# azmyrajab/polars_ols

Hardware: AMD Instinct MI355X
Metric: group_regressions_per_sec (higher is better)
Workload: dtype f32

## Files before the change

polars_ols_amd/csrc/api.hip:

```cpp
#include <algorithm>
#include <cmath>
#include <cctype>
#include <cstdlib>
#include <strings.h>
#include <condition_variable>
#include <mutex>
#include <thread>

#include "common.hpp"
#include "api_internal.hpp"
#include "k1_gram_chol.hpp"
#include "k2_resident.hpp"
#include "k2w_resident.hpp"
#include "k4_rolling.hpp"
#include "k5_enet.hpp"
#include "k6_svd.hpp"
#include "k8_wide.hpp"
#include "k10_ridge_path.hpp"
#include "k11_rlm.hpp"
#include "k13_glm.hpp"
#include "k14_iv.hpp"
#include "k12_enet_cv.hpp"
#include "dyn_prep.hpp"

// ... 118 lines not shown
    const uint64_t sum = ((h0 * 31 + h1) * 31 + h2) * 31 + h3;
    const bool hit = ctx->offsets.valid && ctx->offs_n == n_groups && ctx->offs_sum == sum &&
                     ctx->offs_copy.size() == (size_t)cnt && std::memcmp(ctx->offs_copy.data(), offs, bytes) == 0;
    if (!hit) {
        void *dptr = nullptr;
        ctx->offsets.valid = false;
        int rc = grow(ctx->offsets, bytes, &dptr);
        if (rc) return rc;
        if ((rc = upload_small(ctx, dptr, offs, bytes))) return rc;
        ctx->offsets.valid = true;
        ctx->offs_copy.assign(offs, offs + cnt);
        ctx->offs_n = n_groups;
        ctx->offs_sum = sum;
        ctx->offs_id++;
    }
    ctx->offs_host = offs;
    ctx->offs_generation = generation;
    ctx->offs_max_rows = sc.max_rows;
    ctx->offs_min_rows = sc.min_rows;
    ctx->offs_small_mask = sc.small_mask;
    std::memcpy(ctx->offs_hist_cnt, sc.hist_cnt, sizeof(sc.hist_cnt));
    std::memcpy(ctx->offs_hist_rows, sc.hist_rows, sizeof(sc.hist_rows));
    ctx->offs_wave_overflow = sc.wave_overflow;
    ctx->offs_tail_group = sc.tail_group;
    ctx->offs_aligned[0] = sc.aligned[0];
    ctx->offs_aligned[1] = sc.aligned[1];
    *d_offs = static_cast<const int64_t *>(ctx->offsets.buf.ptr);
    *max_rows = sc.max_rows;
    return POLS_OK;
}

static bool ieq(const char *a, const char *b) {
    for (; *a && *b; ++a, ++b)
        if (std::tolower((unsigned char)*a) != std::tolower((unsigned char)*b)) return false;
    return *a == *b;
}

bool options_set(Options &o, const char *key, const char *v) {
    if (!key) return false;
    if (!strncasecmp(key, "POLS_", 5)) key += 5;
    const bool on = v != nullptr;
    const Options d;
    if (ieq(key, "TIMELINE")) o.timeline = on;
    else if (ieq(key, "K1_NOOCC4")) o.k1_noocc4 = on;
    else if (ieq(key, "K1_NOFAST")) o.k1_nofast = on;
    else if (ieq(key, "K1_NOEDGE")) o.k1_noedge = on;
    else if (ieq(key, "K1_NOTINY")) o.k1_notiny = on;
    else if (ieq(key, "K1_NORC1")) o.k1_norc1 = on;
    else if (ieq(key, "K1_SHAPE")) { o.k1_shape_team = on && ieq(v, "team"); o.k1_shape_wave = on && ieq(v, "wave"); }
    else if (ieq(key, "K1_F64_TEAM")) o.k1_f64_team256 = on && std::atoi(v) == 256;
    else if (ieq(key, "KG_NOYV")) o.kg_noyv = on;
    else if (ieq(key, "KG_SINGLE_BUFFER")) o.kg_single_buffer = on;
    else if (ieq(key, "NO_CLASSES")) o.no_classes = on;
    else if (ieq(key, "PREDICT_LOOP")) o.predict_loop = on;
    else if (ieq(key, "K2_NOPREFETCH")) o.k2_noprefetch = on;
    else if (ieq(key, "NO_SPLIT")) o.no_split = on;
    else if (ieq(key, "K1_PASSES")) o.k1_passes = on ? std::atoi(v) : d.k1_passes;
    else if (ieq(key, "K1_WG")) o.k1_wg = on ? std::atoi(v) : d.k1_wg;
    else if (ieq(key, "K1T_RC4")) o.k1t_rc4 = on ? (std::atoi(v) != 0) : d.k1t_rc4;
    else if (ieq(key, "K1T_SUB8")) o.k1t_sub8 = on ? std::atoi(v) : d.k1t_sub8;
    else if (ieq(key, "K1_NT_LOADS")) o.k1_nt_loads = on ? (std::atoi(v) != 0) : d.k1_nt_loads;
    else if (ieq(key, "K1_XCD")) o.k1_xcd = on ? std::atoi(v) : d.k1_xcd;
    else if (ieq(key, "K4P_LPS")) o.k4p_lps = on ? std::atoi(v) : d.k4p_lps;
    else if (ieq(key, "SEG_TARGET")) o.seg_target = on ? std::atoi(v) : d.seg_target;
    else if (ieq(key, "K1_RC2_WIDE")) o.k1_rc2_wide = on ? std::atoi(v) != 0 : d.k1_rc2_wide;
    else if (ieq(key, "DEBUG_SKIP_FIXUP")) o.debug_skip_fixup = on && std::atoi(v) != 0;
    else if (ieq(key, "K1_PERSIST")) o.k1_persist = on ? (std::atoi(v) != 0) : d.k1_persist;
    else if (ieq(key, "K1_PERSIST_SUB")) o.k1_persist_sub = on ? std::atoi(v) : d.k1_persist_sub;
    else if (ieq(key, "K1T_SUB32")) o.k1t_sub32 = on ? (std::atoi(v) != 0) : d.k1t_sub32;
    else if (ieq(key, "STATIC_ENGINE")) o.static_engine = !on ? 0 : ieq(v, "stream") ? 1 : ieq(v, "k2") ? 2 : ieq(v, "nok2") ? 3 : ieq(v, "k2w") ? 4 : 0;
    else if (ieq(key, "RLS_ENGINE")) o.rls_engine = !on ? RlsEngine::Auto : ieq(v, "seq") ? RlsEngine::Seq : ieq(v, "scan") ? RlsEngine::Scan : ieq(v, "chunk") ? RlsEngine::Chunk : ieq(v, "halo") ? RlsEngine::Halo : RlsEngine::Auto;
    else if (ieq(key, "RLM_ENGINE")) o.rlm_engine = !on ? 0 : ieq(v, "stream") ? 1 : 0;
    else if (ieq(key, "GLM_ENGINE")) o.glm_engine = !on ? 0 : ieq(v, "split") ? 1 : 0;
    else if (ieq(key, "ABSORB2_ROUTE")) o.absorb2_route = !on ? 0 : ieq(v, "global") ? 1 : 0;
    else if (ieq(key, "RANDOM_EFFECTS_ROUTE")) o.random_effects_route = !on ? 0 : ieq(v, "global") ? 1 : 0;
    else if (ieq(key, "RLS_SPINS")) o.rls_spin_limit = on ? std::atoi(v) : d.rls_spin_limit;
    else if (ieq(key, "RLS_EARLY")) o.rls_early = on ? std::atoi(v) : d.rls_early;
    else if (ieq(key, "ROLLING_ENGINE")) {
        using E = RollingEngine;
        o.rolling_engine = !on ? E::Auto : ieq(v, "chunk") ? E::Chunk : ieq(v, "halo") ? E::Halo : ieq(v, "nocompact") ? E::NoCompact : ieq(v, "halowave") ? E::HaloWave : ieq(v, "scatter") ? E::Scatter : E::Auto;
    }
    else if (ieq(key, "K1_ENGINE")) o.k1_engine = !on ? 0 : ieq(v, "valu") ? 1 : ieq(v, "mfma") ? 2 : 0;
    else if (ieq(key, "K9_TAKE")) o.k9_take = !on ? 0 : ieq(v, "gather") ? 1 : ieq(v, "scatter") ? 2 : 0;
    else return false;
    return true;
}

void options_from_env(Options &o) {
    static const char *const keys[] = {"TIMELINE", "K1_NOOCC4", "K1_NOFAST", "K1_NOTINY", "K1_NORC1", "K1_SHAPE", "K1_F64_TEAM",
                                       "KG_NOYV", "K2_NOPREFETCH", "K1_PASSES", "K1_WG", "RLS_SPINS", "RLS_EARLY", "K1T_RC4", "K1_NT_LOADS", "STATIC_ENGINE",
                                       "RLS_ENGINE", "RLM_ENGINE", "GLM_ENGINE", "ABSORB2_ROUTE", "RANDOM_EFFECTS_ROUTE", "ROLLING_ENGINE", "K1_ENGINE", "K9_TAKE", "K1_PERSIST", "K1_PERSIST_SUB", "K1T_SUB32", "K1_NOEDGE", "K1T_SUB8",
                                       "K1_XCD", "NO_SPLIT", "DEBUG_SKIP_FIXUP", "K4P_LPS", "SEG_TARGET", "K1_RC2_WIDE", "KG_SINGLE_BUFFER", "PREDICT_LOOP", "NO_CLASSES"};
    char name[64];
    for (const char *k : keys) {
        std::snprintf(name, sizeof(name), "POLS_%s", k);
        if (const char *v = std::getenv(name)) options_set(o, k, v);
    }
}

static bool timing_sampled(pols_ctx *ctx) {
    if (!ctx->timing) return false;
    return (ctx->timing_tick++ % ctx->timing_stride) == 0;
}

void timing_begin(pols_ctx *ctx) {
    ctx->timing_open = false;
    if (!timing_sampled(ctx)) return;
    ctx->timing_open = true;
    if (ctx->timed_used == ctx->timed.size()) {
        TimedLaunch t;
        if (hipEventCreate(&t.start) != hipSuccess || hipEventCreate(&t.stop) != hipSuccess) return;
        ctx->timed.push_back(t);
    }
    hipEventRecord(ctx->timed[ctx->timed_used].start, ctx->stream);
}

bool timing_pair(pols_ctx *ctx, hipEvent_t *start, hipEvent_t *stop) {
    if (!timing_sampled(ctx)) return false;
    if (ctx->timed_used == ctx->timed.size()) {
        TimedLaunch t;
        if (hipEventCreate(&t.start) != hipSuccess || hipEventCreate(&t.stop) != hipSuccess) return false;
        ctx->timed.push_back(t);
    }
    *start = ctx->timed[ctx->timed_used].start;
    *stop = ctx->timed[ctx->timed_used].stop;
    ctx->timed_used++;
    return true;
}

void timing_end(pols_ctx *ctx) {
    if (!ctx->timing_open || ctx->timed_used >= ctx->timed.size()) return;
    ctx->timing_open = false;
    hipEventRecord(ctx->timed[ctx->timed_used].stop, ctx->stream);
    ctx->timed_used++;
}

int check_ctx(pols_ctx *ctx) {
    if (!ctx) return fail(POLS_ERR_INVALID, "ctx is NULL");
    POLS_HIP(hipSetDevice(ctx->device));
    return POLS_OK;
}


template <typename T>
__global__ void __launch_bounds__(256) null_weights_kernel(const T *w, T *out, int64_t n) {
    using V = typename Vec16<T>::type;
    constexpr int VN = Vec16<T>::N;
    const int64_t i0 = ((int64_t)blockIdx.x * 256 + threadIdx.x) * VN;
    if (i0 + VN <= n) {
        const V v = *reinterpret_cast<const V *>(w + i0);
        T f[4];
#pragma unroll
        for (int e = 0; e < VN; ++e) { const T x = vget<T>(v, e); f[e] = x != x ? (T)1e-24 : x; }
        if constexpr (VN == 4) *reinterpret_cast<V *>(out + i0) = V{f[0], f[1], f[2], f[3]};
        else *reinterpret_cast<V *>(out + i0) = V{f[0], f[1]};
    } else {
        for (int64_t i = i0; i < n; ++i) { const T x = w[i]; out[i] = x != x ? (T)1e-24 : x; }
    }
}

int fill_null_weights(pols_ctx *ctx, const pols_batch *b, Staged *st) {
    if (!st->w || b->null_free || b->n_rows <= 0) return POLS_OK;
    void *dst = const_cast<void *>(st->w);
    if (b->mem == POLS_MEM_DEVICE) {
        int rc = ensure_scratch(ctx, Work::NullWeights, round256(dtype_size(b->dtype) * (size_t)b->n_rows), &dst);
        if (rc) return rc;
    }
    const int vn = b->dtype == POLS_F32 ? 4 : 2;
    const unsigned blocks = (unsigned)((b->n_rows + 256 * (int64_t)vn - 1) / (256 * (int64_t)vn));
    if (b->dtype == POLS_F32) hipLaunchKernelGGL(null_weights_kernel<float>, dim3(blocks), dim3(256), 0, ctx->stream, static_cast<const float *>(st->w), static_cast<float *>(dst), b->n_rows);
    else hipLaunchKernelGGL(null_weights_kernel<double>, dim3(blocks), dim3(256), 0, ctx->stream, static_cast<const double *>(st->w), static_cast<double *>(dst), b->n_rows);
    POLS_HIP(hipGetLastError());
    st->w = dst;
    return POLS_OK;
// ... 170 lines not shown
    if (same_frame) extra_per_seg = std::max<size_t>(extra_per_seg, sc.nz2);
    sc.valid = false;
    std::vector<int64_t> so;
    std::vector<int32_t> sm, sf((size_t)n_items + 1);
    if (!ids) so.push_back(0);
    int64_t max_len = 0, max_seg = 0;
    for (int64_t i = 0; i < n_items; ++i) {
        const int64_t g = ids ? (int64_t)(*ids)[(size_t)i] : i;
        if (i > 0) max_seg = std::max<int64_t>(max_seg, (int64_t)sm.size() - sf[(size_t)i - 1]);
        sf[(size_t)i] = (int32_t)sm.size();
        const int64_t s0 = b->group_offsets[g], e0 = b->group_offsets[g + 1];
        const int64_t pieces = std::max<int64_t>(1, (e0 - s0 + seg_target - 1) / seg_target);
        const int64_t len = std::max<int64_t>(1, ((e0 - s0 + pieces - 1) / pieces + 255) / 256 * 256);
        max_len = std::max(max_len, std::min(len, e0 - s0));
        for (int64_t r = s0; r < e0 || r == s0; r += len) {
            if (ids) so.push_back(r);
            so.push_back(std::min(e0, r + len));
            sm.push_back((int32_t)i);
            if (e0 == s0) break;
        }
    }
    sf[(size_t)n_items] = (int32_t)sm.size();
    if (n_items > 0) max_seg = std::max<int64_t>(max_seg, (int64_t)sm.size() - sf[(size_t)n_items - 1]);
    const int64_t n_seg = (int64_t)sm.size();
    seg_tables_layout(cv, *t, n_seg, n_items, ids != nullptr, extra_per_seg);
    if ((rc = carve(sc, cv))) return rc;
    if ((rc = upload_small(ctx, const_cast<int64_t *>(t->offs), so.data(), sizeof(int64_t) * so.size()))) return rc;
    if ((rc = upload_small(ctx, const_cast<int32_t *>(t->map), sm.data(), sizeof(int32_t) * sm.size()))) return rc;
    if ((rc = upload_small(ctx, const_cast<int32_t *>(t->first), sf.data(), sizeof(int32_t) * sf.size()))) return rc;
    sc.valid = true; sc.offs_id = ctx->offs_id; sc.n_groups = b->n_groups; sc.n_rows = b->n_rows; sc.seg_target = seg_target;
    sc.class_key = class_key; sc.n_items = n_items;
    sc.n_seg = n_seg; sc.nz2 = extra_per_seg; sc.nulls = false; sc.max_len = max_len; sc.max_seg = max_seg;
    t->max_len = max_len; t->max_seg = max_seg;
    return POLS_OK;
}

extern "C" {

int pols_device_count(void) {
    int n = 0;
    if (hipGetDeviceCount(&n) != hipSuccess) return 0;
    return n;
}

const char *pols_version(void) { return "pols_mi355x 0.1.0 (gfx950)"; }
const char *pols_last_error(void) { return g_err; }

int pols_create(int device_id, pols_ctx **out) {
    if (!out) return fail(POLS_ERR_INVALID, "out is NULL");
    *out = nullptr;
    int n = 0;
    if (hipGetDeviceCount(&n) != hipSuccess || n <= 0)
        return fail(POLS_ERR_NO_DEVICE, "no HIP device visible; libpols_mi355x has no CPU fallback");
    if (device_id < 0 || device_id >= n) return fail(POLS_ERR_INVALID, "device_id %d out of range [0, %d)", device_id, n);
    POLS_HIP(hipSetDevice(device_id));
    hipDeviceProp_t prop;
    POLS_HIP(hipGetDeviceProperties(&prop, device_id));
    if (std::strncmp(prop.gcnArchName, "gfx950", 6) != 0)
        return fail(POLS_ERR_NO_DEVICE, "device %d is %s; this library carries gfx950 code objects only", device_id, prop.gcnArchName);
    pols_ctx *ctx = new pols_ctx();
    ctx->device = device_id;
    ctx->num_cus = prop.multiProcessorCount;
    if (hipStreamCreateWithFlags(&ctx->own_stream, hipStreamNonBlocking) != hipSuccess) {
        delete ctx;
        return fail(POLS_ERR_HIP, "hipStreamCreate failed");
    }
    ctx->stream = ctx->own_stream;
    options_from_env(ctx->opt);
    *out = ctx;
    return POLS_OK;
}

int pols_set_option(pols_ctx *ctx, const char *key, const char *value) {
    if (!ctx || !key) return fail(POLS_ERR_INVALID, "ctx / key is NULL");
    if (!options_set(ctx->opt, key, value)) return fail(POLS_ERR_INVALID, "unknown option '%s'", key);
    return POLS_OK;
}

void pols_destroy(pols_ctx *ctx) {
    if (!ctx) return;
    hipSetDevice(ctx->device);
    hipStreamSynchronize(ctx->stream);
    for (DeviceBuffer *d : {&ctx->offsets.buf, &ctx->chunk_cache.buf, &ctx->k3c.buf, &ctx->k3h.buf, &ctx->class_cache.buf, &ctx->seg_cache[0].buf,
                            &ctx->seg_cache[1].buf, &ctx->start_flags.buf, &ctx->k3c_gran, &ctx->k4c_fix})
        if (d->ptr) hipFree(d->ptr);
    for (auto &d : ctx->work)
        if (d.ptr) hipFree(d.ptr);
    if (ctx->fb_flag) hipFree(ctx->fb_flag);
    for (auto &t : ctx->timed) { hipEventDestroy(t.start); hipEventDestroy(t.stop); }
    for (auto &ps : ctx->pinned) {
        if (ps.done) hipEventDestroy(ps.done);
        if (ps.ptr) hipHostFree(ps.ptr);
    }
    if (ctx->switch_event) hipEventDestroy(ctx->switch_event);
    if (ctx->own_stream) hipStreamDestroy(ctx->own_stream);
    delete ctx;
}

int pols_set_stream(pols_ctx *ctx, void *hip_stream) {
    if (!ctx) return fail(POLS_ERR_INVALID, "ctx is NULL");
    hipStream_t next = static_cast<hipStream_t>(hip_stream);
    if (next != ctx->stream) {
        if (!ctx->switch_event) POLS_HIP(hipEventCreateWithFlags(&ctx->switch_event, hipEventDisableTiming));
        POLS_HIP(hipEventRecord(ctx->switch_event, ctx->stream));
        POLS_HIP(hipStreamWaitEvent(next, ctx->switch_event, 0));
    }
    ctx->stream = next;
    return POLS_OK;
}

int pols_use_private_stream(pols_ctx *ctx) {
    if (!ctx) return fail(POLS_ERR_INVALID, "ctx is NULL");
    return pols_set_stream(ctx, ctx->own_stream);
}

int pols_synchronize(pols_ctx *ctx) {
    int rc = check_ctx(ctx);
    if (rc) return rc;
    POLS_HIP(hipStreamSynchronize(ctx->stream));
    return POLS_OK;
}

int pols_timing_enable(pols_ctx *ctx, int enable) {
    if (!ctx) return fail(POLS_ERR_INVALID, "ctx is NULL");
    ctx->timing = enable != 0;
    ctx->timing_stride = enable > 1 ? enable : 1;
    ctx->timing_tick = 0;
    ctx->timed_used = 0;
    return POLS_OK;
}

int pols_timing_collect(pols_ctx *ctx, float *ms_out, int max) {
    if (!ctx || !ms_out) return fail(POLS_ERR_INVALID, "NULL argument");
    if (hipStreamSynchronize(ctx->stream) != hipSuccess) return fail(POLS_ERR_HIP, "stream sync failed");
    int n = 0;
    for (size_t i = 0; i < ctx->timed_used && n < max; ++i) {
        float ms = 0.f;
        if (hipEventElapsedTime(&ms, ctx->timed[i].start, ctx->timed[i].stop) == hipSuccess) ms_out[n++] = ms;
    }
    ctx->timed_used = 0;
    return n;
}

const char *pols_last_kernel_name(pols_ctx *ctx) { return ctx ? ctx->last_kernel.c_str() : ""; }

void pols_ols_params_default(pols_ols_params *p) {
    std::memset(p, 0, sizeof(*p));
    p->alpha = 0.0;
    p->has_l1_ratio = 0;
    p->max_iter = 1000;
    p->tol = 1.0e-5;
    p->positive = 0;
    p->solve_method = POLS_SOLVE_AUTO;
    p->has_rcond = 0;
    p->null_policy = POLS_NULL_IGNORE;
}

int pols_predict(pols_ctx *ctx, const pols_batch *b, const void *coef, int64_t coef_rows, void *pred_out) {
    return pols_predict_policy(ctx, b, coef, coef_rows, POLS_NULL_IGNORE, pred_out);
}

int pols_predict_policy(pols_ctx *ctx, const pols_batch *b, const void *coef, int64_t coef_rows, int32_t null_policy, void *pred_out) {
    int rc = check_ctx(ctx);
    if (rc) return rc;
    pols_out o;
    std::memset(&o, 0, sizeof(o));
    o.pred = pred_out;
// ... 276 lines not shown
```

polars_ols_amd/csrc/api_static.hip:

```cpp
#include <algorithm>
#include <cmath>
#include <cstring>
#include <string>

#include "common.hpp"
#include "api_internal.hpp"
#include "k1_gram_chol.hpp"
#include "k2_resident.hpp"
#include "k2w_resident.hpp"
#include "k5_enet.hpp"
#include "k6_svd.hpp"
#include "k8_wide.hpp"
#include "../../include/pols_mi355x_debug.h"

namespace pols {
template <typename T> bool k1m_fits(int k_user, bool has_w, int64_t max_rows);

int resolve_solve_plan(const pols_ols_params *p, int dtype, int kt, int n_targets, SolvePlan *out) {
    const int m = p->solve_method;
    const double alpha = p->alpha;
    const bool positive = p->positive != 0, multi = n_targets > 1;
    SolvePlan s;
    if (alpha == 0.0 && !positive && (m == POLS_SOLVE_AUTO || m == POLS_SOLVE_SVD || m == POLS_SOLVE_QR)) {
        s.branch = SolveBranch::Ols;
// ... 476 lines not shown
    if (!p) return fail(POLS_ERR_INVALID, "params is NULL");
    StaticCall c{ctx, b, p, o};
    if ((rc = effective_null_policy(b, p, &c.pol))) return rc;
    c.kt = b->n_features + (b->add_intercept ? 1 : 0);
    if ((rc = resolve_solve_plan(p, b->dtype, c.kt, 1, &c.plan))) return rc;
    if (b->n_groups == 0) return POLS_OK;
    if (c.kt > 31) {
        if (info) return fail(POLS_ERR_INVALID, "internal: the wide statistics path calls wide_static itself");
        return wide_static(ctx, b, p, o, c.kt, c.plan);
    }
    if ((rc = upload_offsets(ctx, b->group_offsets, b->n_groups, &c.d_offs, &c.max_rows, b->offsets_generation))) return rc;
    if ((rc = stage_inputs(ctx, b, b->n_groups, c.kt, o, &c.st))) return rc;
    if ((rc = fill_null_weights(ctx, b, &c.st))) return rc;
    if (!c.plan.enet()) {
        if (!c.st.status) {
            void *sp = nullptr;
            if ((rc = ensure_scratch(ctx, Work::Status, sizeof(int32_t) * (size_t)b->n_groups, &sp))) return rc;
            c.st.status = static_cast<int32_t *>(sp);
        }
        if ((rc = ensure_fallback_epoch(ctx))) return rc;
    }
    const RoutePick r = pick_static_route(route_inputs(ctx->opt, b, p, c.pol, c.plan, c.max_rows, ctx->offs_aligned, ctx->offs_hist_cnt, ctx->offs_hist_rows));
    switch (r.route) {
        case StaticRoute::Wide: return fail(POLS_ERR_INVALID, "internal: wide frames leave before the route picker");
        case StaticRoute::SvdAll: rc = route_svd_all(c); break;
        case StaticRoute::K2: rc = route_k2(c); break;
        case StaticRoute::K2w: rc = route_k2w(c); break;
        case StaticRoute::Streamed: rc = route_streamed(c); break;
        case StaticRoute::ClassesStreamedTop: rc = route_classes_streamed_top(c, r); break;
        case StaticRoute::Classes:
        case StaticRoute::K1: rc = route_k1(c, r); break;
    }
    if (rc) return rc;
    if (!info) return unstage_outputs(ctx, b, b->n_groups, c.kt, o, c.st);
    info->st = c.st; info->d_offs = c.d_offs; info->gram = c.stream_gram;
    return POLS_OK;
}

int wide_static(pols_ctx *ctx, const pols_batch *b, const pols_ols_params *p, pols_out *o, int kt, const SolvePlan &plan,
                const void *const *y_cols, int m, void *const *pred_cols, WideInfo *info) {
    int rc;
    const bool enet = plan.enet();
    const int64_t *d_offs = nullptr;
    int64_t max_rows = 0;
    if ((rc = upload_offsets(ctx, b->group_offsets, b->n_groups, &d_offs, &max_rows, b->offsets_generation))) return rc;
    Staged st;
    if ((rc = stage_inputs(ctx, b, b->n_groups * m, kt, o, &st))) return rc;
    if ((rc = fill_null_weights(ctx, b, &st))) return rc;
    const size_t G = (size_t)b->n_groups;
    const int NZ = kt + m, nt = (NZ + 63) / 64, npairs = nt * (nt + 1) / 2;
    std::vector<const void *> yptr;
    std::vector<void *> pptr;
    const bool host = b->mem == POLS_MEM_HOST;
    const size_t colb_mt = round256(dtype_size(b->dtype) * (size_t)b->n_rows);
    if (m > 1) {
        yptr.assign(y_cols, y_cols + m);
        if (pred_cols) pptr.assign(pred_cols, pred_cols + m);
        if (host) {
            char *ys = nullptr, *ps = nullptr;
            Carve mt;
            mt.keep(ys, colb_mt * (size_t)m);
            if (pred_cols) mt.keep(ps, colb_mt * (size_t)m);
            if ((rc = carve(ctx, Work::HostStaged, mt))) return rc;
            for (int t = 0; t < m; ++t) {
                char *yt = column(ys, colb_mt, (size_t)t);
                POLS_HIP(hipMemcpyAsync(yt, y_cols[t], dtype_size(b->dtype) * (size_t)b->n_rows, hipMemcpyHostToDevice, ctx->stream));
                yptr[t] = yt;
                if (pred_cols) pptr[t] = column(ps, colb_mt, (size_t)t);
            }
        }
    }
    const size_t mat = sizeof(double) * (size_t)NZ * NZ;
    int64_t splits = std::max<int64_t>(1, (2048 + (int64_t)G * npairs - 1) / ((int64_t)G * npairs));
    splits = std::min<int64_t>(splits, std::max<int64_t>(1, (max_rows + 255) / 256));
    while (splits > 1 && (double)splits * (double)G * (double)mat > 2e9) splits /= 2;
    int64_t rps = (std::max<int64_t>(1, max_rows) + splits - 1) / splits;
    rps = (rps + 63) / 64 * 64;
    splits = (std::max<int64_t>(1, max_rows) + rps - 1) / rps;

    void *tab = nullptr;
    std::vector<const void *> table(st.x.begin(), st.x.end());
    table.insert(table.end(), yptr.begin(), yptr.end());
    table.insert(table.end(), pptr.begin(), pptr.end());
    if ((rc = ensure_scratch(ctx, Work::Tables, sizeof(void *) * table.size(), &tab))) return rc;
    if ((rc = upload_small(ctx, tab, table.data(), sizeof(void *) * table.size()))) return rc;
    const bool nulls = p->null_policy != POLS_NULL_IGNORE;
    WideArgs a;
    std::memset(&a, 0, sizeof(a));
    Carve cv;
    cv.keep(a.gram, mat * G);
    cv.keep(a.partial, mat * G * (size_t)splits);
    cv.keep(a.coef64, sizeof(double) * G * kt * m);
    if (nulls) {
        cv.keep(a.rowmask, (size_t)b->n_rows);
        cv.keep(a.nfit, sizeof(double) * G);
    }
    if ((rc = carve(ctx, Work::Gram, cv))) return rc;
    if (!st.status) {
        void *sp = nullptr;
        if ((rc = ensure_scratch(ctx, Work::Status, sizeof(int32_t) * G, &sp))) return rc;
        st.status = static_cast<int32_t *>(sp);
    }
    if ((rc = ensure_fallback_epoch(ctx))) return rc;

    a.cols = static_cast<const void *const *>(tab);
    if (m > 1) {
        a.n_targets = m;
        a.ycols = a.cols + b->n_features;
        if (!pptr.empty()) a.pred_cols = static_cast<void *const *>(tab) + b->n_features + m;
    }
    a.y = st.y; a.w = st.w; a.offs = d_offs; a.n_groups = b->n_groups; a.n_rows = b->n_rows;
    a.k_user = b->n_features; a.kt = kt;
    a.splits = (int32_t)splits; a.rows_per_split = rps;
    a.alpha = enet ? p->alpha : plan.ridge_alpha; a.l1_ratio = plan.enet_l1; a.tol = p->tol; a.max_iter = p->max_iter;
    a.positive = p->positive ? 1 : 0; a.active_set = (p->solve_method == POLS_SOLVE_CD_ACTIVE_SET) ? 1 : 0;
    a.pivot_tol = plan.pivot_tol;
    a.rc_factor = plan.rc_factor;
    a.status = st.status; a.fb_flag = ctx->fb_flag; a.epoch = ctx->epoch;
    a.coef = st.coef; a.pred = st.pred; a.resid = st.resid;
    a.null_policy = p->null_policy;
    if (nulls) {
        a.valid = st.valid;
        if ((rc = wide_rowmask_launch(ctx, b->dtype, a))) return rc;
    }
    if ((rc = wide_gram_launch(ctx, b->dtype, a))) return rc;
    if (enet) {
        if ((rc = wide_cd_launch(ctx, b->dtype, a))) return rc;
    } else {
        a.fix_mode = plan.fix_mode;
        if ((rc = wide_chol_launch(ctx, b->dtype, a))) return rc;
        int workers = (int)std::min<size_t>(G, 64);
        void *wk = nullptr;
        const bool lu = fix_uses_lu(a.fix_mode);
        const int64_t ncmax = lu ? kt : std::min<int64_t>(std::max<int64_t>(1, max_rows), kt);
        a.work_w_elems = (int64_t)(kt + m) * std::max<int64_t>(1, max_rows);
        a.work_stride = a.work_w_elems + ncmax * ncmax + 2 * ncmax + (lu ? (int64_t)kt * m : 0);
        while (workers > 1 && (double)workers * (double)a.work_stride * 8.0 > 1e9) workers /= 2;
        if ((rc = ensure_scratch(ctx, Work::Fixup, sizeof(double) * (size_t)workers * (size_t)a.work_stride, &wk))) return rc;
        a.work = static_cast<double *>(wk);
        if ((rc = wide_minnorm_launch(ctx, b->dtype, a, workers))) return rc;
    }
    if (st.pred || st.resid || a.pred_cols)
        if ((rc = wide_predict_launch(ctx, b->dtype, a))) return rc;
    if (m > 1 && host && pred_cols)
        for (int t = 0; t < m; ++t)
            POLS_HIP(hipMemcpyAsync(pred_cols[t], pptr[t], dtype_size(b->dtype) * (size_t)b->n_rows, hipMemcpyDeviceToHost, ctx->stream));
    if (info) { info->st = st; info->a = a; return POLS_OK; }
    return unstage_outputs(ctx, b, b->n_groups * m, kt, o, st);
}

}

using namespace pols;

extern "C" {

int pols_least_squares(pols_ctx *ctx, const pols_batch *b, const pols_ols_params *p, pols_out *o) {
    return ls_core(ctx, b, p, o, nullptr);
}

int pols_multi_target_least_squares(pols_ctx *ctx, const pols_batch *b, const void *const *y_cols, int32_t n_targets,
                                    const pols_ols_params *p, void *const *pred_cols, void *coef, int32_t *status) {
    int rc = check_ctx(ctx);
    if (rc) return rc;
    if (!b || !p || !y_cols) return fail(POLS_ERR_INVALID, "batch / params / y_cols is NULL");
    if (n_targets < 1 || n_targets > 256) return fail(POLS_ERR_INVALID, "n_targets must be in 1..256");
    for (int t = 0; t < n_targets; ++t)
        if (!y_cols[t] || (pred_cols && !pred_cols[t])) return fail(POLS_ERR_INVALID, "target / prediction column %d is NULL", t);
// ... 98 lines not shown
```

polars_ols_amd/csrc/common.hpp:

```cpp
#pragma once

#include <hip/hip_runtime.h>
#include <hip/hip_ext.h>

#include <atomic>
#include <cstdarg>
#include <cstdint>
#include <cstdio>
#include <cstring>
#include <string>
#include <vector>

#include "../../include/pols_mi355x.h"

namespace pols {

void set_error(const char *fmt, ...);
int fail(int code, const char *fmt, ...);

#define POLS_HIP(call)                                                                       \
    do {                                                                                     \
        hipError_t e_ = (call);                                                              \
        if (e_ != hipSuccess)                                                                \
            return ::pols::fail(POLS_ERR_HIP, "%s failed: %s (%s:%d)", #call, hipGetErrorString(e_), \
// ... 64 lines not shown
    AbsorbIds,
    AbsorbIndex,
    AbsorbCats,
    AbsorbMoments,
    AbsorbOut,
    Absorb2Ids,
    Absorb2Order,
    Absorb2Index,
    Absorb2Cats,
    Absorb2Cols,
    Absorb2Moments,
    Absorb2Out,
    GlsarMoments,
    GlsarState,
    GlsarOut,
    RandomEffectsIds,
    RandomEffectsIndex,
    RandomEffectsCats,
    RandomEffectsMoments,
    RandomEffectsOut,
    Count
};

struct TimedLaunch {
    hipEvent_t start, stop;
};

enum class RollingEngine {
    Auto,
    Chunk,
    Halo,
    NoCompact,
    HaloWave,
    Scatter,
};
enum class RlsEngine {
    Auto,
    Seq,
    Scan,
    Chunk,
    Halo,
};

struct Options {
    bool timeline = false;
    bool k1_noocc4 = false;
    bool k1_nofast = false;
    bool k1_notiny = false;
    bool k1_norc1 = false;
    bool k1_shape_team = false;
    bool k1_shape_wave = false;
    bool k1_f64_team256 = false;
    bool no_classes = false;
    bool kg_single_buffer = false;
    bool predict_loop = false;
    bool kg_noyv = false;
    int k1_passes = 0;
    int k1t_rc4 = -1;
    int k1t_sub8 = -1;
    int static_engine = 0;
    RlsEngine rls_engine = RlsEngine::Auto;
    int rls_early = 0;
    int rls_spin_limit = -1;
    RollingEngine rolling_engine = RollingEngine::Auto;
    int k1_engine = 0;
    int k9_take = 0;
    int k1_nt_loads = -1;
    bool no_split = false;
    bool k2_noprefetch = false;
    bool k1_noedge = false;
    int k1t_sub32 = -1;
    int k1_persist_sub = 0;
    int k1_persist = -1;
    bool debug_skip_fixup = false;
    bool k1_rc2_wide = true;
    int seg_target = 0;
    int k4p_lps = 0;
    int k1_wg = 0;
    int rlm_engine = 0;
    int glm_engine = 0;
    int absorb2_route = 0;
    int random_effects_route = 0;
    int k1_xcd = 0;
};
void options_from_env(Options &o);
bool options_set(Options &o, const char *key, const char *value);

}

struct pols_ctx {
    int device = 0;
    hipStream_t own_stream = nullptr;
    hipStream_t stream = nullptr;
    hipEvent_t switch_event = nullptr;
    int num_cus = 0;
    pols::DeviceBuffer work[(int)pols::Work::Count];
    pols::Options opt;
    bool timing = false;
    int timing_stride = 1;
    int timing_tick = 0;
    bool timing_open = false;
    std::vector<pols::TimedLaunch> timed;
    size_t timed_used = 0;
    std::string last_kernel;
    pols::CachedTable offsets;
    const int64_t *offs_host = nullptr;
    uint64_t offs_generation = 0;
    std::vector<int64_t> offs_copy;
    int64_t offs_n = -1;
    uint64_t offs_sum = 0;
    uint64_t offs_id = 0;
    struct PinnedSlot { void *ptr = nullptr; size_t cap = 0; hipEvent_t done = nullptr; bool busy = false; };
    PinnedSlot pinned[4];
    int pinned_next = 0;
    int64_t offs_max_rows = 0;
    int64_t offs_min_rows = 0;
    int64_t offs_hist_cnt[48] = {0}, offs_hist_rows[48] = {0};
    int32_t offs_small_mask = 0;
    int64_t offs_tail_group = -1;
    int64_t offs_wave_overflow = 0;
    int32_t *fb_flag = nullptr;
    int32_t epoch = 0;
    bool offs_aligned[2] = {false, false};
    struct : pols::CachedTable { uint64_t offs_id = 0; int64_t n_groups = -1, n_rows = -1, mp = -1, n_chunks = 0; int32_t chunk_len = 0; } chunk_cache;
    struct : pols::CachedTable { uint64_t offs_id = 0; int64_t n_groups = -1, n_rows = -1, tile_rows = 0, n_tiles = 0; } k3c;
    struct : pols::CachedTable { uint64_t offs_id = 0; int64_t n_groups = -1, n_rows = -1, tile_rows = 0; } k3h;
    struct : pols::CachedTable { uint64_t offs_id = 0; int64_t cut[3] = {0, 0, 0}, n[4] = {0, 0, 0, 0}; int n_cut = 0;
                                 std::vector<int32_t> host_last; } class_cache;
    struct : pols::CachedTable { uint64_t offs_id = 0; int64_t n_groups = -1, n_rows = -1, seg_target = 0, n_seg = 0, max_len = 0, max_seg = 0, class_key = 0, n_items = 0; size_t nz2 = 0; bool nulls = false; } seg_cache[2];
    struct : pols::CachedTable { uint64_t offs_id = 0; int64_t n_groups = -1, n_rows = -1; } start_flags;
    pols::DeviceBuffer k3c_gran;
    unsigned long long k3c_epoch = 0;
    pols::DeviceBuffer k4c_fix;
    uint64_t k4c_fix_turn = 0;
};

namespace pols {

int grow(DeviceBuffer &b, size_t bytes, void **out, bool *fresh = nullptr);
int grow(CachedTable &t, size_t bytes, void **out);
int ensure_scratch(pols_ctx *ctx, Work w, size_t bytes, void **out);
int upload_offsets(pols_ctx *ctx, const int64_t *offs, int64_t n_groups, const int64_t **d_offs, int64_t *max_rows,
                   uint64_t generation = 0);
int upload_small(pols_ctx *ctx, void *dst_device, const void *src, size_t bytes);
void timing_begin(pols_ctx *ctx);
void timing_end(pols_ctx *ctx);
bool timing_pair(pols_ctx *ctx, hipEvent_t *start, hipEvent_t *stop);
int report_timeline(pols_ctx *ctx, const unsigned long long *d_dbg, int64_t n_groups, int n_stamps, const char *name);

inline size_t dtype_size(int dtype) { return dtype == POLS_F32 ? 4 : 8; }
inline size_t round256(size_t b) { return (b + 255) & ~(size_t)255; }

struct OncePerDevice {
    std::atomic<uint64_t> mask{0};
    bool needed(int device) const { return (mask.load(std::memory_order_acquire) & (1ull << (device & 63))) == 0; }
    void done(int device) { mask.fetch_or(1ull << (device & 63), std::memory_order_release); }
};

#if defined(__HIPCC__)

template <int CTRL, int ROW_MASK>
__device__ __forceinline__ int dpp_mov(int v) {
    return __builtin_amdgcn_update_dpp(0, v, CTRL, ROW_MASK, 0xf, false);
}

template <int CTRL, int ROW_MASK = 0xf>
__device__ __forceinline__ float dpp_get(float v) {
    return __int_as_float(dpp_mov<CTRL, ROW_MASK>(__float_as_int(v)));
}

template <int CTRL, int ROW_MASK = 0xf>
__device__ __forceinline__ double dpp_get(double v) {
    const long long b = __double_as_longlong(v);
    const int lo = dpp_mov<CTRL, ROW_MASK>((int)(b & 0xffffffffLL));
    const int hi = dpp_mov<CTRL, ROW_MASK>((int)(b >> 32));
    return __longlong_as_double(((long long)hi << 32) | (unsigned int)lo);
}

template <typename T>
__device__ __forceinline__ T wave_sum_row3(T v) {
    v += dpp_get<0xB1>(v);
    v += dpp_get<0x4E>(v);
    v += dpp_get<0x141>(v);
    v += dpp_get<0x140>(v);
    v += dpp_get<0x142, 0xa>(v);
    v += dpp_get<0x143, 0xc>(v);
    return v;
}

__device__ __forceinline__ void pair_halves(float &a, float b) {
    const auto r = __builtin_amdgcn_permlane32_swap(__float_as_uint(a), __float_as_uint(b), false, false);
    a = __uint_as_float(r[0]) + __uint_as_float(r[1]);
}
__device__ __forceinline__ void pair_halves(double &a, double b) {
    const unsigned long long ba = __double_as_longlong(a), bb = __double_as_longlong(b);
    const auto lo = __builtin_amdgcn_permlane32_swap((unsigned)ba, (unsigned)bb, false, false);
    const auto hi = __builtin_amdgcn_permlane32_swap((unsigned)(ba >> 32), (unsigned)(bb >> 32), false, false);
    a = __longlong_as_double(((unsigned long long)hi[0] << 32) | lo[0]) +
        __longlong_as_double(((unsigned long long)hi[1] << 32) | lo[1]);
}
__device__ __forceinline__ void pair_rows(float &a, float b) {
    const auto r = __builtin_amdgcn_permlane16_swap(__float_as_uint(a), __float_as_uint(b), false, false);
    a = __uint_as_float(r[0]) + __uint_as_float(r[1]);
}
__device__ __forceinline__ void pair_rows(double &a, double b) {
    const unsigned long long ba = __double_as_longlong(a), bb = __double_as_longlong(b);
    const auto lo = __builtin_amdgcn_permlane16_swap((unsigned)ba, (unsigned)bb, false, false);
    const auto hi = __builtin_amdgcn_permlane16_swap((unsigned)(ba >> 32), (unsigned)(bb >> 32), false, false);
    a = __longlong_as_double(((unsigned long long)hi[0] << 32) | lo[0]) +
        __longlong_as_double(((unsigned long long)hi[1] << 32) | lo[1]);
}
template <typename T>
__device__ __forceinline__ T row_allreduce(T v) {
// ... 95 lines not shown
```

polars_ols_amd/csrc/k8_wide.hip:

```cpp
#include "k8_wide.hpp"
#include "fix_solvers.inl"
#include "k1m_kernel.inl"
#include "k7_stats.hpp"

namespace pols {

constexpr int WG_TS = 64;
constexpr int WG_RS = 65;

template <typename T>
__device__ __forceinline__ double wide_z(const WideArgs &a, const void *colp, int z, int64_t r) {
    const int ku = a.k_user, kt = a.kt;
    if (z < ku) return (double)null_fill<T>(a.null_policy, static_cast<const T *>(colp)[r]);
    if (z >= kt) return (double)null_fill<T>(a.null_policy, static_cast<const T *>(a.ycols ? a.ycols[z - kt] : a.y)[r]);
    if (z == kt - 1 && ku != kt) return 1.0;
    return 0.0;
}

template <typename T>
__global__ void __launch_bounds__(256) wide_rowmask_kernel(const WideArgs a) {
    __shared__ int cnt_s;
    const int64_t g = blockIdx.x;
    const int64_t s = a.offs[g], e = a.offs[g + 1];
    const int pol = a.null_policy;
    if (threadIdx.x == 0) cnt_s = 0;
    __syncthreads();
    int cnt = 0;
    for (int64_t r = s + threadIdx.x; r < e; r += 256) {
        bool fit = true;
        if (null_checks_y(pol)) {
            const T yv = static_cast<const T *>(a.y)[r];
            fit = (yv == yv) && !(a.valid && !a.valid[r]);
            if (fit && null_checks_x(pol))
                for (int j = 0; j < a.k_user && fit; ++j) { const T xv = static_cast<const T *>(a.cols[j])[r]; fit = (xv == xv); }
        }
        a.rowmask[r] = fit ? 1 : 0;
        cnt += fit ? 1 : 0;
    }
    if (cnt) atomicAdd(&cnt_s, cnt);
    __syncthreads();
    if (threadIdx.x == 0) a.nfit[g] = (double)cnt_s;
}

int wide_rowmask_launch(pols_ctx *ctx, int dtype, const WideArgs &a) {
    if (a.n_groups == 0) return POLS_OK;
    if (dtype == POLS_F32) hipLaunchKernelGGL(wide_rowmask_kernel<float>, dim3((unsigned)a.n_groups), dim3(256), 0, ctx->stream, a);
    else hipLaunchKernelGGL(wide_rowmask_kernel<double>, dim3((unsigned)a.n_groups), dim3(256), 0, ctx->stream, a);
    POLS_HIP(hipGetLastError());
    return POLS_OK;
}

template <typename T>
__global__ void __launch_bounds__(256) wide_gram_kernel(const WideArgs a) {
    using M = Mfma16<double>;
    __shared__ double Zi[WG_TS * WG_RS], Zj[WG_TS * WG_RS];
    __shared__ double sw_s[WG_TS];
    __shared__ const void *cp_i[WG_TS], *cp_j[WG_TS];
    const int tid = threadIdx.x, lane = tid & 63, wv = tid >> 6;
    const int NZ = a.kt + wide_m(a), nt = (NZ + WG_TS - 1) / WG_TS;
    int ti = 0, rem = blockIdx.x;
    while (rem >= nt - ti) { rem -= nt - ti; ++ti; }
    const int tj = ti + rem;
    const int64_t g = blockIdx.y;
    const int64_t s = a.offs[g], e = a.offs[g + 1];
    const int64_t r_begin = s + (int64_t)blockIdx.z * a.rows_per_split;
    const int64_t r_end = min(e, r_begin + a.rows_per_split);
    if (r_begin >= r_end) return;
    if (tid < WG_TS) {
        const int zi = WG_TS * ti + tid, zj = WG_TS * tj + tid;
        cp_i[tid] = zi < a.k_user ? a.cols[zi] : nullptr;
        cp_j[tid] = zj < a.k_user ? a.cols[zj] : nullptr;
    }
    M::acc_t acc[4];
#pragma unroll
    for (int t = 0; t < 4; ++t) acc[t] = M::acc_t{0, 0, 0, 0};
    const double *ZJ = (ti == tj) ? Zi : Zj;
    for (int64_t r0 = r_begin; r0 < r_end; r0 += WG_TS) {
        const int rows_here = (int)min((int64_t)WG_TS, r_end - r0);
        __syncthreads();
        if (tid < WG_TS) {
            double swv = tid < rows_here ? (a.w ? sqrt((double)static_cast<const T *>(a.w)[r0 + tid]) : 1.0) : 0.0;
            if (a.rowmask && tid < rows_here && !a.rowmask[r0 + tid]) swv = 0.0;
            sw_s[tid] = swv;
        }
        __syncthreads();
        for (int idx = tid; idx < WG_TS * WG_TS; idx += 256) {
            const int c = idx >> 6, r = idx & 63;
            const bool in = r < rows_here;
            const int zi = WG_TS * ti + c;
            Zi[c * WG_RS + r] = (in && zi < NZ) ? wide_z<T>(a, cp_i[c], zi, r0 + r) * sw_s[r] : 0.0;
            if (ti != tj) {
                const int zj = WG_TS * tj + c;
                Zj[c * WG_RS + r] = (in && zj < NZ) ? wide_z<T>(a, cp_j[c], zj, r0 + r) * sw_s[r] : 0.0;
            }
        }
        __syncthreads();
        const int zc = lane & 15, kq = lane >> 4;
        const double *ap = Zi + (16 * wv + zc) * WG_RS + kq;
        const double *bp = ZJ + zc * WG_RS + kq;
#pragma unroll 4
        for (int rr = 0; rr < WG_TS; rr += 4) {
            const double av = ap[rr];
#pragma unroll
            for (int t = 0; t < 4; ++t) acc[t] = M::mma(av, bp[16 * t * WG_RS + rr], acc[t]);
        }
    }
    double *P = a.partial + ((size_t)blockIdx.z * a.n_groups + g) * NZ * NZ;
    const int dcol = lane & 15;
#pragma unroll
    for (int t = 0; t < 4; ++t)
#pragma unroll
        for (int reg = 0; reg < 4; ++reg) {
            const int i = WG_TS * ti + 16 * wv + (lane >> 4) + 4 * reg, j = WG_TS * tj + 16 * t + dcol;
            if (i < NZ && j < NZ) P[(size_t)i * NZ + j] = acc[t][reg];
        }
}

__global__ void __launch_bounds__(256) wide_reduce_kernel(const WideArgs a) {
    const int NZ = a.kt + wide_m(a);
    const int64_t g = blockIdx.y;
    const int64_t n = a.offs[g + 1] - a.offs[g];
    const int nsp = (int)((n + a.rows_per_split - 1) / a.rows_per_split);
    const size_t mat = (size_t)NZ * NZ;
    for (size_t q = (size_t)blockIdx.x * 256 + threadIdx.x; q < mat; q += (size_t)gridDim.x * 256) {
        int i = (int)(q / NZ), j = (int)(q - (size_t)i * NZ);
        if (i / WG_TS > j / WG_TS) { const int t = i; i = j; j = t; }
        double v = 0.0;
        for (int sp = 0; sp < nsp; ++sp) v += a.partial[((size_t)sp * a.n_groups + g) * mat + (size_t)i * NZ + j];
        a.gram[(size_t)g * mat + q] = v;
    }
}

int wide_gram_launch(pols_ctx *ctx, int dtype, const WideArgs &a) {
    const int NZ = a.kt + wide_m(a), nt = (NZ + WG_TS - 1) / WG_TS, npairs = nt * (nt + 1) / 2;
    char name[64];
    std::snprintf(name, sizeof(name), "k8_wide_gram_%s_k%d", dtype == POLS_F32 ? "f32" : "f64", a.kt);
    ctx->last_kernel = name;
    timing_begin(ctx);
    const dim3 grid((unsigned)npairs, (unsigned)a.n_groups, (unsigned)a.splits);
    if (dtype == POLS_F32) hipLaunchKernelGGL(wide_gram_kernel<float>, grid, dim3(256), 0, ctx->stream, a);
    else hipLaunchKernelGGL(wide_gram_kernel<double>, grid, dim3(256), 0, ctx->stream, a);
    const unsigned rb = (unsigned)std::min<size_t>(1024, ((size_t)NZ * NZ + 255) / 256);
    hipLaunchKernelGGL(wide_reduce_kernel, dim3(rb, (unsigned)a.n_groups), dim3(256), 0, ctx->stream, a);
    timing_end(ctx);
    POLS_HIP(hipGetLastError());
    return POLS_OK;
}

template <int NV>
__device__ __forceinline__ void wide_block_sum(double (&v)[NV], double *red, int nwaves) {
    const int lane = threadIdx.x & 63, wv = threadIdx.x >> 6;
    __syncthreads();
#pragma unroll
    for (int i = 0; i < NV; ++i) {
        const double sacc = wave_sum_row3(v[i]);
        if (lane == 63) red[i * nwaves + wv] = sacc;
    }
    __syncthreads();
#pragma unroll
    for (int i = 0; i < NV; ++i) {
        double t = 0.0;
        for (int w = 0; w < nwaves; ++w) t += red[i * nwaves + w];
        v[i] = t;
    }
}

template <typename T, int NTHREADS, bool IN_LDS>
__global__ void __launch_bounds__(NTHREADS) wide_chol_kernel(const WideArgs a) {
    extern __shared__ double a_lds[];
    constexpr int KCAP = IN_LDS ? 128 : K8_KMAX;
    __shared__ double xs[KCAP], dinv[KCAP], diag0[KCAP];
    __shared__ int ok_s;
    constexpr int NW = NTHREADS / 64;
    const int tid = threadIdx.x, lane = tid & 63, wv = tid >> 6;
    const int kt = a.kt, m = wide_m(a), NZ = kt + m;
    const int64_t g = blockIdx.x;
    const int64_t n = a.nfit ? (int64_t)a.nfit[g] : a.offs[g + 1] - a.offs[g];
    double *Gm = a.gram + (size_t)g * NZ * NZ;
    const int LD = IN_LDS ? (NZ | 1) : NZ;
    double *A = IN_LDS ? a_lds : Gm;
    if (IN_LDS) {
        for (int q = tid; q < NZ * NZ; q += NTHREADS) { const int i = q / NZ, c = q - i * NZ; if (c <= i) A[i * LD + c] = Gm[q]; }
        __syncthreads();
    }
    for (int i = tid; i < kt; i += NTHREADS) { const double d0 = A[(size_t)i * LD + i] + a.alpha; A[(size_t)i * LD + i] = d0; diag0[i] = d0; }
    if (tid == 0) ok_s = 1;
    __syncthreads();
    for (int j = 0; j < kt; ++j) {
        const double d = A[(size_t)j * LD + j];
        const double di = 1.0 / d;
        if (tid == 0) { dinv[j] = di; if (!(d > a.pivot_tol * diag0[j])) ok_s = 0; }
        const double *cj = A + j;
        for (int i = j + 1 + wv; i < NZ; i += NW) {
            const double li = cj[(size_t)i * LD] * di;
            double *row = A + (size_t)i * LD;
            const int cmax = (i >= kt) ? kt - 1 : i;
            for (int c = j + 1 + lane; c <= cmax; c += 64) row[c] -= li * cj[(size_t)c * LD];
        }
        __syncthreads();
    }
    const bool by_shape = n < (int64_t)kt && a.alpha == 0.0 && (a.fix_mode == FIX_OLS_AUTO || a.fix_mode == FIX_MINNORM);
    int st = POLS_GROUP_OK;
    if (n == 0) st = POLS_GROUP_EMPTY;
    else if (!ok_s || by_shape) { st = POLS_GROUP_FALLBACK; if (tid == 0 && a.fb_flag) *a.fb_flag = a.epoch; }
    for (int t = 0; t < m; ++t) {
        __syncthreads();
        for (int i = tid; i < kt; i += NTHREADS) xs[i] = A[(size_t)(kt + t) * LD + i];
        __syncthreads();
        for (int j = kt - 1; j >= 0; --j) {
            const double xj = xs[j] * dinv[j];
            const double *row = A + (size_t)j * LD;
            for (int i = tid; i < j; i += NTHREADS) xs[i] -= row[i] * xj;
            __syncthreads();
            if (tid == 0) xs[j] = xj;
        }
        __syncthreads();
        for (int i = tid; i < kt; i += NTHREADS) {
            const double out = (n == 0) ? 0.0 : xs[i];
            if (a.coef) static_cast<T *>(a.coef)[((size_t)g * m + t) * kt + i] = (T)out;
            a.coef64[((size_t)g * m + t) * kt + i] = out;
        }
    }
    if (tid == 0 && a.status) a.status[g] = st;
}

template <typename T>
// ... 387 lines not shown
```

Before: 132.3 million.

## Prefetch next row tile in wide Gram kernel and cache pointer table

Rewrites the wide Gram kernel so each thread keeps column pointers in registers and software-prefetches the next 64-row tile into registers while the current tile's MFMA products run, replacing the shared-memory pointer staging. The split-reduce kernel now batches eight partial loads per iteration to expose memory-level parallelism. The device pointer table is cached across calls and re-uploaded only when the host pointers change, avoiding a host-to-device copy per call. The old path stays available behind a legacy option. In exchange the kernel holds 32 more values per thread in registers, which may lower occupancy.

Measured after the change: 132.8 million (median of 2 runs). No clear change (+0.3%).

```diff
diff --git a/polars_ols_amd/csrc/api.hip b/polars_ols_amd/csrc/api.hip
--- a/polars_ols_amd/csrc/api.hip
+++ b/polars_ols_amd/csrc/api.hip
@@ -224,6 +224,7 @@
     }
     else if (ieq(key, "K1_ENGINE")) o.k1_engine = !on ? 0 : ieq(v, "valu") ? 1 : ieq(v, "mfma") ? 2 : 0;
     else if (ieq(key, "K9_TAKE")) o.k9_take = !on ? 0 : ieq(v, "gather") ? 1 : ieq(v, "scatter") ? 2 : 0;
+    else if (ieq(key, "WIDE_ENGINE")) o.wide_engine = !on ? 0 : ieq(v, "legacy") ? 1 : 0;
     else return false;
     return true;
 }
@@ -231,7 +232,7 @@
 void options_from_env(Options &o) {
     static const char *const keys[] = {"TIMELINE", "K1_NOOCC4", "K1_NOFAST", "K1_NOTINY", "K1_NORC1", "K1_SHAPE", "K1_F64_TEAM",
                                        "KG_NOYV", "K2_NOPREFETCH", "K1_PASSES", "K1_WG", "RLS_SPINS", "RLS_EARLY", "K1T_RC4", "K1_NT_LOADS", "STATIC_ENGINE",
-                                       "RLS_ENGINE", "RLM_ENGINE", "GLM_ENGINE", "ABSORB2_ROUTE", "RANDOM_EFFECTS_ROUTE", "ROLLING_ENGINE", "K1_ENGINE", "K9_TAKE", "K1_PERSIST", "K1_PERSIST_SUB", "K1T_SUB32", "K1_NOEDGE", "K1T_SUB8",
+                                       "RLS_ENGINE", "RLM_ENGINE", "GLM_ENGINE", "ABSORB2_ROUTE", "RANDOM_EFFECTS_ROUTE", "ROLLING_ENGINE", "K1_ENGINE", "K9_TAKE", "WIDE_ENGINE", "K1_PERSIST", "K1_PERSIST_SUB", "K1T_SUB32", "K1_NOEDGE", "K1T_SUB8",
                                        "K1_XCD", "NO_SPLIT", "DEBUG_SKIP_FIXUP", "K4P_LPS", "SEG_TARGET", "K1_RC2_WIDE", "KG_SINGLE_BUFFER", "PREDICT_LOOP", "NO_CLASSES"};
     char name[64];
     for (const char *k : keys) {
@@ -568,7 +569,7 @@
     hipSetDevice(ctx->device);
     hipStreamSynchronize(ctx->stream);
     for (DeviceBuffer *d : {&ctx->offsets.buf, &ctx->chunk_cache.buf, &ctx->k3c.buf, &ctx->k3h.buf, &ctx->class_cache.buf, &ctx->seg_cache[0].buf,
-                            &ctx->seg_cache[1].buf, &ctx->start_flags.buf, &ctx->k3c_gran, &ctx->k4c_fix})
+                            &ctx->seg_cache[1].buf, &ctx->start_flags.buf, &ctx->wide_table.buf, &ctx->k3c_gran, &ctx->k4c_fix})
         if (d->ptr) hipFree(d->ptr);
     for (auto &d : ctx->work)
         if (d.ptr) hipFree(d.ptr);
diff --git a/polars_ols_amd/csrc/api_static.hip b/polars_ols_amd/csrc/api_static.hip
--- a/polars_ols_amd/csrc/api_static.hip
+++ b/polars_ols_amd/csrc/api_static.hip
@@ -582,8 +582,19 @@
     std::vector<const void *> table(st.x.begin(), st.x.end());
     table.insert(table.end(), yptr.begin(), yptr.end());
     table.insert(table.end(), pptr.begin(), pptr.end());
-    if ((rc = ensure_scratch(ctx, Work::Tables, sizeof(void *) * table.size(), &tab))) return rc;
-    if ((rc = upload_small(ctx, tab, table.data(), sizeof(void *) * table.size()))) return rc;
+    if (ctx->opt.wide_engine == 1) {
+        if ((rc = ensure_scratch(ctx, Work::Tables, sizeof(void *) * table.size(), &tab))) return rc;
+        if ((rc = upload_small(ctx, tab, table.data(), sizeof(void *) * table.size()))) return rc;
+    } else {
+        auto &wt = ctx->wide_table;
+        if ((rc = grow(wt, sizeof(void *) * table.size(), &tab))) return rc;
+        if (!wt.valid || wt.host != table) {
+            wt.valid = false;
+            if ((rc = upload_small(ctx, tab, table.data(), sizeof(void *) * table.size()))) return rc;
+            wt.host = table;
+            wt.valid = true;
+        }
+    }
     const bool nulls = p->null_policy != POLS_NULL_IGNORE;
     WideArgs a;
     std::memset(&a, 0, sizeof(a));
diff --git a/polars_ols_amd/csrc/common.hpp b/polars_ols_amd/csrc/common.hpp
--- a/polars_ols_amd/csrc/common.hpp
+++ b/polars_ols_amd/csrc/common.hpp
@@ -170,6 +170,7 @@
     int absorb2_route = 0;
     int random_effects_route = 0;
     int k1_xcd = 0;
+    int wide_engine = 0;
 };
 void options_from_env(Options &o);
 bool options_set(Options &o, const char *key, const char *value);
@@ -217,6 +218,7 @@
                                  std::vector<int32_t> host_last; } class_cache;
     struct : pols::CachedTable { uint64_t offs_id = 0; int64_t n_groups = -1, n_rows = -1, seg_target = 0, n_seg = 0, max_len = 0, max_seg = 0, class_key = 0, n_items = 0; size_t nz2 = 0; bool nulls = false; } seg_cache[2];
     struct : pols::CachedTable { uint64_t offs_id = 0; int64_t n_groups = -1, n_rows = -1; } start_flags;
+    struct : pols::CachedTable { std::vector<const void *> host; } wide_table;
     pols::DeviceBuffer k3c_gran;
     unsigned long long k3c_epoch = 0;
     pols::DeviceBuffer k4c_fix;
diff --git a/polars_ols_amd/csrc/k8_wide.hip b/polars_ols_amd/csrc/k8_wide.hip
--- a/polars_ols_amd/csrc/k8_wide.hip
+++ b/polars_ols_amd/csrc/k8_wide.hip
@@ -7,6 +7,8 @@
 
 constexpr int WG_TS = 64;
 constexpr int WG_RS = 65;
+
+static bool wide_legacy(const pols_ctx *ctx) { return ctx->opt.wide_engine == 1; }
 
 template <typename T>
 __device__ __forceinline__ double wide_z(const WideArgs &a, const void *colp, int z, int64_t r) {
@@ -51,7 +53,7 @@
 }
 
 template <typename T>
-__global__ void __launch_bounds__(256) wide_gram_kernel(const WideArgs a) {
+__global__ void __launch_bounds__(256) wide_gram_legacy_kernel(const WideArgs a) {
     using M = Mfma16<double>;
     __shared__ double Zi[WG_TS * WG_RS], Zj[WG_TS * WG_RS];
     __shared__ double sw_s[WG_TS];
@@ -116,7 +118,7 @@
         }
 }
 
-__global__ void __launch_bounds__(256) wide_reduce_kernel(const WideArgs a) {
+__global__ void __launch_bounds__(256) wide_reduce_legacy_kernel(const WideArgs a) {
     const int NZ = a.kt + wide_m(a);
     const int64_t g = blockIdx.y;
     const int64_t n = a.offs[g + 1] - a.offs[g];
@@ -131,6 +133,123 @@
     }
 }
 
+template <typename T>
+__device__ __forceinline__ void wide_gram_cols(const WideArgs &a, int NZ, int tile, int wv, const T *(&p)[16]) {
+#pragma unroll
+    for (int k = 0; k < 16; ++k) {
+        const int z = WG_TS * tile + wv + 4 * k;
+        const void *q = nullptr;
+        if (z < a.k_user) q = a.cols[z];
+        else if (z >= a.kt && z < NZ) q = a.ycols ? a.ycols[z - a.kt] : a.y;
+        p[k] = static_cast<const T *>(q);
+    }
+}
+
+template <typename T>
+__device__ __forceinline__ T wide_gload(const T *p, int64_t r) { return ((const __attribute__((address_space(1))) T *)p)[r]; }
+
+template <typename T>
+__device__ __forceinline__ void wide_gram_fetch(const T *const (&p)[16], int64_t r, T (&v)[16]) {
+#pragma unroll
+    for (int k = 0; k < 16; ++k) v[k] = p[k] ? wide_gload<T>(p[k], r) : T(0);
+}
+
+template <typename T>
+__device__ __forceinline__ void wide_gram_stage(const WideArgs &a, int NZ, int tile, int wv, int lane, bool in, double sw,
+                                                const T *const (&p)[16], const T (&v)[16], double *Z) {
+#pragma unroll
+    for (int k = 0; k < 16; ++k) {
+        const int c = wv + 4 * k, z = WG_TS * tile + c;
+        double x = 0.0;
+        if (in && z < NZ) x = (p[k] ? (double)null_fill<T>(a.null_policy, v[k]) : (z == a.kt - 1 && a.k_user != a.kt) ? 1.0 : 0.0) * sw;
+        Z[c * WG_RS + lane] = x;
+    }
+}
+
+template <typename T>
+__global__ void __launch_bounds__(256) wide_gram_kernel(const WideArgs a) {
+    using M = Mfma16<double>;
+    __shared__ double Zi[WG_TS * WG_RS], Zj[WG_TS * WG_RS];
+    const int tid = threadIdx.x, lane = tid & 63, wv = __builtin_amdgcn_readfirstlane(tid >> 6);
+    const int NZ = a.kt + wide_m(a), nt = (NZ + WG_TS - 1) / WG_TS;
+    int ti = 0, rem = blockIdx.x;
+    while (rem >= nt - ti) { rem -= nt - ti; ++ti; }
+    const int tj = ti + rem;
+    const int64_t g = blockIdx.y;
+    const int64_t s = a.offs[g], e = a.offs[g + 1];
+    const int64_t r_begin = s + (int64_t)blockIdx.z * a.rows_per_split;
+    const int64_t r_end = min(e, r_begin + a.rows_per_split);
+    if (r_begin >= r_end) return;
+    const bool two = ti != tj;
+    const T *pi[16], *pj[16];
+    wide_gram_cols<T>(a, NZ, ti, wv, pi);
+    wide_gram_cols<T>(a, NZ, tj, wv, pj);
+    T vi[16], vj[16], wr = T(1);
+    uint8_t fit = 1;
+    auto fetch = [&](int64_t r0) {
+        const int64_t r = min(r0 + lane, r_end - 1);
+        wide_gram_fetch<T>(pi, r, vi);
+        if (two) wide_gram_fetch<T>(pj, r, vj);
+        if (a.w) wr = static_cast<const T *>(a.w)[r];
+        if (a.rowmask) fit = a.rowmask[r];
+    };
+    fetch(r_begin);
+    M::acc_t acc[4];
+#pragma unroll
+    for (int t = 0; t < 4; ++t) acc[t] = M::acc_t{0, 0, 0, 0};
+    const double *ZJ = two ? Zj : Zi;
+    for (int64_t r0 = r_begin; r0 < r_end; r0 += WG_TS) {
+        const bool in = r0 + lane < r_end;
+        double sw = in ? (a.w ? sqrt((double)wr) : 1.0) : 0.0;
+        if (a.rowmask && in && !fit) sw = 0.0;
+        __syncthreads();
+        wide_gram_stage<T>(a, NZ, ti, wv, lane, in, sw, pi, vi, Zi);
+        if (two) wide_gram_stage<T>(a, NZ, tj, wv, lane, in, sw, pj, vj, Zj);
+        __syncthreads();
+        if (r0 + WG_TS < r_end) fetch(r0 + WG_TS);
+        const int zc = lane & 15, kq = lane >> 4;
+        const double *ap = Zi + (16 * wv + zc) * WG_RS + kq;
+        const double *bp = ZJ + zc * WG_RS + kq;
+#pragma unroll 4
+        for (int rr = 0; rr < WG_TS; rr += 4) {
+            const double av = ap[rr];
+#pragma unroll
+            for (int t = 0; t < 4; ++t) acc[t] = M::mma(av, bp[16 * t * WG_RS + rr], acc[t]);
+        }
+    }
+    double *P = a.partial + ((size_t)blockIdx.z * a.n_groups + g) * NZ * NZ;
+    const int dcol = lane & 15;
+#pragma unroll
+    for (int t = 0; t < 4; ++t)
+#pragma unroll
+        for (int reg = 0; reg < 4; ++reg) {
+            const int i = WG_TS * ti + 16 * wv + (lane >> 4) + 4 * reg, j = WG_TS * tj + 16 * t + dcol;
+            if (i < NZ && j < NZ) P[(size_t)i * NZ + j] = acc[t][reg];
+        }
+}
+
+__global__ void __launch_bounds__(256) wide_reduce_kernel(const WideArgs a) {
+    const int NZ = a.kt + wide_m(a);
+    const int64_t g = blockIdx.y;
+    const int64_t n = a.offs[g + 1] - a.offs[g];
+    const int nsp = (int)((n + a.rows_per_split - 1) / a.rows_per_split);
+    const size_t mat = (size_t)NZ * NZ;
+    for (size_t q = (size_t)blockIdx.x * 256 + threadIdx.x; q < mat; q += (size_t)gridDim.x * 256) {
+        int i = (int)(q / NZ), j = (int)(q - (size_t)i * NZ);
+        if (i / WG_TS > j / WG_TS) { const int t = i; i = j; j = t; }
+        const double *src = a.partial + (size_t)g * mat + (size_t)i * NZ + j;
+        double v = 0.0;
+        for (int sp0 = 0; sp0 < nsp; sp0 += 8) {
+            double t[8];
+#pragma unroll
+            for (int u = 0; u < 8; ++u) t[u] = src[(size_t)min(sp0 + u, nsp - 1) * a.n_groups * mat];
+#pragma unroll
+            for (int u = 0; u < 8; ++u) if (sp0 + u < nsp) v += t[u];
+        }
+        a.gram[(size_t)g * mat + q] = v;
+    }
+}
+
 int wide_gram_launch(pols_ctx *ctx, int dtype, const WideArgs &a) {
     const int NZ = a.kt + wide_m(a), nt = (NZ + WG_TS - 1) / WG_TS, npairs = nt * (nt + 1) / 2;
     char name[64];
@@ -138,10 +257,11 @@
     ctx->last_kernel = name;
     timing_begin(ctx);
     const dim3 grid((unsigned)npairs, (unsigned)a.n_groups, (unsigned)a.splits);
-    if (dtype == POLS_F32) hipLaunchKernelGGL(wide_gram_kernel<float>, grid, dim3(256), 0, ctx->stream, a);
-    else hipLaunchKernelGGL(wide_gram_kernel<double>, grid, dim3(256), 0, ctx->stream, a);
+    const bool legacy = wide_legacy(ctx);
+    if (dtype == POLS_F32) hipLaunchKernelGGL(legacy ? wide_gram_legacy_kernel<float> : wide_gram_kernel<float>, grid, dim3(256), 0, ctx->stream, a);
+    else hipLaunchKernelGGL(legacy ? wide_gram_legacy_kernel<double> : wide_gram_kernel<double>, grid, dim3(256), 0, ctx->stream, a);
     const unsigned rb = (unsigned)std::min<size_t>(1024, ((size_t)NZ * NZ + 255) / 256);
-    hipLaunchKernelGGL(wide_reduce_kernel, dim3(rb, (unsigned)a.n_groups), dim3(256), 0, ctx->stream, a);
+    hipLaunchKernelGGL(legacy ? wide_reduce_legacy_kernel : wide_reduce_kernel, dim3(rb, (unsigned)a.n_groups), dim3(256), 0, ctx->stream, a);
     timing_end(ctx);
     POLS_HIP(hipGetLastError());
     return POLS_OK;
```
